# NGoetz/NF

Measured on NVIDIA B200. Metric: nis_flow_fwd_logdet_points_per_sec, higher is better.
Workload: dtype f32

## Files before the change

nf_b200/csrc/flow_fwd.cu:

```cuda
#include <stdlib.h>
#include "common.cuh"
#include "spline.cuh"
#include <cooperative_groups.h>
#include "flow_fwd_common.cuh"

__global__ void flow_pack_kernel(DevFlow F, const float* __restrict__ params, const float* __restrict__ bn_running,
                                 float* __restrict__ wpack, int bn_mode) {
    const int c = blockIdx.y;
    const DevCell& q = F.cells[c];
    const float* p = params + q.param_off;
    float* pk = wpack + q.pk_off;
    const int tid = blockIdx.x * blockDim.x + threadIdx.x, nth = gridDim.x * blockDim.x;
    if (bn_mode == NIS_BN_EVAL) {
        const float* rs = bn_running + q.bn_off;
        for (int l = 0; l <= F.depth; ++l) {
            const int W = F.W(c, l), Wp = F.Wp(c, l);
            const long long g = F.p_bn_gamma(c, l), r = F.r_mean(c, l);
            for (int j = tid; j < Wp; j += nth) {
                float sc = 0.f, sh = 0.f;
                if (j < W) {
                    sc = p[g + j] / sqrtf(rs[r + W + j] + F.eps);
                    sh = p[g + W + j] - rs[r + j] * sc;
                }
                pk[q.aff_off[l] + j] = sc;
// ... 196 lines not shown
template <int NT>
__global__ void __launch_bounds__(NT) flow_fwd_coop_kernel(const __grid_constant__ DevFlow F, const FwdArgs A0) {
    extern __shared__ __align__(16) float sm[];
    cooperative_groups::grid_group grid = cooperative_groups::this_grid();
    const long long rows = A0.B * (F.d + 1);
    FwdArgs A = A0;
    for (int c = 0; c < F.n_cells; ++c) {
        A.c_begin = c; A.c_end = c + 1;
        A.from_state = c > 0;
        A.state_in = c > 0 ? (A0.saved ? A0.saved + (long long)c * rows : A0.scratch_state) : nullptr;
        A.state_out = nullptr; A.to_out = 0;
        for (int l = 0; l <= F.depth; ++l) {
            A.stats_layer = l;
            fwd_generic_body<NT>(F, A, sm);
            grid.sync();
        }
        const bool last = c == F.n_cells - 1;
        A.stats_layer = -1;
        A.to_out = last;
        A.state_out = A0.saved ? A0.saved + (long long)(c + 1) * rows : (last ? nullptr : A0.scratch_state);
        fwd_generic_body<NT>(F, A, sm);
    }
}

size_t nis_flow_bwd_scratch_floats(const DevFlow& F, int64_t B);
bool nis_tiled_supported(const DevFlow& F, int64_t B);
size_t nis_tiled_zbuf_floats(int64_t B);
bool nis_tc_supported(const DevFlow& F, int64_t B, int bn_mode);
int nis_tc_pack(const DevFlow& F, const float* params, float* tcpack, cudaStream_t s);
int nis_launch_tc(const DevFlow& F, const FwdArgs& A, const float* tcpack, cudaStream_t s);
bool nis_tc_split_eval(const DevFlow& F);
bool nis_h_supported(const DevFlow& F, int64_t B, int bn_mode);
int nis_h_pack(const DevFlow& F, const float* params, float* tcpack, cudaStream_t s);
int nis_launch_h(const DevFlow& F, const FwdArgs& A, const float* tcpack, cudaStream_t s);
bool nis_bwd_tc_supported(const DevFlow& F, int64_t B, int bn_mode);
bool nis_wide_supported(const DevFlow& F, int64_t B, int bn_mode);
int nis_wide_pack(const DevFlow& F, const float* params, float* widepack, cudaStream_t s);
int nis_launch_wide(const DevFlow& F, const FwdArgs& A, const float* widepack, cudaStream_t s);
static size_t zbuf_floats(const DevFlow& F, int64_t B) { return nis_tiled_zbuf_floats(B) / 64 * (size_t)(F.maxW > 64 ? F.maxW : 64); }
size_t nis_bwd_tc_scratch_floats(const DevFlow& F, int64_t B);
bool nis_bwd_wide_supported(const DevFlow& F, int64_t B, int bn_mode);
size_t nis_bwd_wide_scratch_floats(const DevFlow& F, int64_t B);
int nis_launch_tiled(const DevFlow& F, const FwdArgs& A, cudaStream_t s);
int nis_launch_col_stats(const DevFlow& F, const FwdArgs& A, cudaStream_t s);
bool nis_moments_supported(const DevFlow& F, int c);
int nis_launch_col_moments(const DevFlow& F, const FwdArgs& A, cudaStream_t s);

#define NIS_TIMING_MAX 512
struct TimingSink { bool on; int n; cudaEvent_t ev[NIS_TIMING_MAX + 1]; int tag[NIS_TIMING_MAX]; bool made; };
static thread_local TimingSink g_timing = {false, 0, {}, {}, false};
static inline void timing_mark(cudaStream_t s, int tag) {
    TimingSink& T = g_timing;
    if (!T.on || T.n >= NIS_TIMING_MAX) return;
    if (tag >= 0) T.tag[T.n++] = tag;
    cudaEventRecord(T.ev[T.n], s);
}
extern "C" int nis_flow_timing_begin(void* stream) {
    TimingSink& T = g_timing;
    if (!T.made) {
        for (int i = 0; i <= NIS_TIMING_MAX; ++i) if (cudaEventCreate(&T.ev[i]) != cudaSuccess) return NIS_ECUDA;
        T.made = true;
    }
    T.on = true; T.n = 0;
    cudaEventRecord(T.ev[0], (cudaStream_t)stream);
    return NIS_OK;
}
extern "C" int nis_flow_timing_end(float* ms, int32_t* tags, int32_t max_n) {
// ... 126 lines not shown
    nis_flow_carve(F, B, workspace, &ws);
    cudaMemsetAsync(ws.counter, 0, 256, s);
    {
        int mx = 0;
        for (int c = 0; c < F.n_cells; ++c) {
            int sz = (c + 1 < F.n_cells ? F.cells[c + 1].pk_off : F.pack_total) - F.cells[c].pk_off;
            if (sz > mx) mx = sz;
        }
        int bx = (mx + 255) / 256;
        if (bx > 64) bx = 64;
        timing_mark(s, -1);
        flow_pack_kernel<<<dim3(bx, F.n_cells), 256, 0, s>>>(F, params, bn_running, ws.wpack, bn_mode);
        NIS_CUDA_CHECK_LAUNCH();
        timing_mark(s, 0);
    }
    FwdArgs A;
    A.in = xj_in; A.in_dtype = in_dtype; A.in_cols = in_cols;
    A.out = xj_out; A.out_dtype = out_dtype;
    A.saved = saved; A.bins = bins_out;
    A.params = params; A.wpack = ws.wpack; A.bn_running = bn_running; A.bn_saved = bn_saved;
    A.partials = ws.partials; A.counter = ws.counter; A.B = B;
    A.zin = nullptr; A.zout = nullptr; A.no_stats = 0; A.z1out = nullptr; A.scratch_state = nullptr; A.inverse = 0; A.zin_layer = 0; A.next_moments = 0;
    const bool tc = nis_tc_supported(F, B, bn_mode);
    const bool hp = tc && nis_h_supported(F, B, bn_mode);
    const bool wide = !tc && nis_wide_supported(F, B, bn_mode);
    const bool tiled = tc || wide || nis_tiled_supported(F, B);
    static const int recompute_env = [] { const char* e = getenv("NIS_TRAIN_RECOMPUTE"); return e ? (e[0] == '1' ? 1 : 0) : -1; }();
    const bool recompute = hp && (recompute_env >= 0 ? recompute_env == 1 : false);
    static const int skip_env = [] { const char* e = getenv("NIS_SKIP_LAST_STORE"); return e && e[0] == '0' ? 0 : 1; }();
    const bool skip_last = hp && !recompute && skip_env && F.depth >= 3 && F.kind == NIS_KIND_PWLIN;
    if (tc) { rc = hp ? nis_h_pack(F, params, ws.tcpack, s) : nis_tc_pack(F, params, ws.tcpack, s); if (rc) return rc; timing_mark(s, 0); }
    if (wide) { rc = nis_wide_pack(F, params, ws.tcpack, s); if (rc) return rc; }
    const long long rows = (long long)B * (F.d + 1);
    if (bn_mode == NIS_BN_EVAL && !tiled) {
        A.state_in = nullptr; A.state_out = nullptr; A.from_state = 0; A.to_out = 1;
        A.c_begin = 0; A.c_end = F.n_cells; A.stats_layer = -1;
        return launch_fwd_any(F, A, s);
    }
    if (bn_mode == NIS_BN_TRAIN && !tiled) {
        static const int coop_env = [] { const char* e = getenv("NIS_COOP"); return e && e[0] == '0' ? 0 : 1; }();
        if (coop_env) {
            A.scratch_state = ws.state;
            A.state_in = nullptr; A.state_out = nullptr; A.from_state = 0; A.to_out = 0;
            A.c_begin = 0; A.c_end = 1; A.stats_layer = 0;
            rc = launch_fwd_coop(F, A, s);
            if (rc == NIS_OK) { timing_mark(s, 2); return NIS_OK; }
        }
    }
    static const int fuse_env = [] { const char* e = getenv("NIS_FUSE_MOMENTS"); return e && e[0] == '0' ? 0 : 1; }();
    bool moments_ready = false;
    float* acts = (wide && bn_mode == NIS_BN_TRAIN && act_saved && saved && nis_act_cache_floats(F, B)) ? act_saved : nullptr;
    const size_t act_layer = (size_t)((B + 127) / 128) * (size_t)F.widths[0] * 128;
    for (int c = 0; c < F.n_cells; ++c) {
        A.c_begin = c; A.c_end = c + 1;
        A.from_state = c > 0;
        A.state_in = c > 0 ? (saved ? saved + (long long)c * rows : ws.state) : nullptr;
        A.state_out = nullptr; A.to_out = 0;
        float* zb[2] = {ws.bwd, ws.bwd + zbuf_floats(F, B)};
        float* const acell = acts ? acts + (size_t)c * F.depth * act_layer : nullptr;
        const bool moments = tiled && bn_mode == NIS_BN_TRAIN && nis_moments_supported(F, c);
        if (bn_mode == NIS_BN_TRAIN) {
            int l0 = 0;
            if (moments) {
                if (!moments_ready) {
                    A.stats_layer = 0;
                    rc = nis_launch_col_moments(F, A, s);
                    if (rc) return rc;
                    timing_mark(s, 1);
                }
                l0 = 2;
            }
            for (int l = l0; l <= F.depth; ++l) {
                A.stats_layer = l;
                if (tiled && l >= 1) {
                    A.zin = (l >= 2 && !(moments && l == 2) && !recompute) ? zb[(l - 1) & 1] : nullptr;
                    A.zout = (recompute || (skip_last && moments && l == F.depth)) ? nullptr : zb[l & 1];
                    if (acell) {
                        if (A.zin) A.zin = acell + (size_t)(l - 2) * act_layer;
                        A.zout = acell + (size_t)(l - 1) * act_layer;
                        A.z1out = (!A.zin && l == 2) ? acell : nullptr;
                    }
                    rc = hp ? nis_launch_h(F, A, ws.tcpack, s) : tc ? nis_launch_tc(F, A, ws.tcpack, s)
                            : wide ? nis_launch_wide(F, A, ws.tcpack, s) : nis_launch_tiled(F, A, s);
                } else if (tiled && l == 0) {
                    rc = nis_launch_col_stats(F, A, s);
                } else {
                    rc = launch_fwd_any(F, A, s);
                }
                if (rc) return rc;
                timing_mark(s, (tc || wide) && l >= 1 ? 10 + 1 + (A.zin ? 2 : 0) : 2);
            }
        }
        A.stats_layer = -1;
        A.zin = (tiled && bn_mode == NIS_BN_TRAIN && !(moments && F.depth == 1) && !recompute) ? zb[F.depth & 1] : nullptr;
        A.zout = nullptr;
        if (acell) { A.zin = acell + (size_t)(F.depth - 1) * act_layer; A.z1out = nullptr; }
        if (skip_last && moments && bn_mode == NIS_BN_TRAIN) { A.zin = zb[(F.depth - 1) & 1]; A.zin_layer = F.depth - 1; }
        if (tc && !hp && bn_mode == NIS_BN_EVAL && nis_tc_split_eval(F)) {
            A.stats_layer = F.depth; A.no_stats = 1; A.zin = nullptr; A.zout = zb[F.depth & 1];
            rc = nis_launch_tc(F, A, ws.tcpack, s);
            if (rc) return rc;
            A.stats_layer = -1; A.no_stats = 0; A.zin = zb[F.depth & 1]; A.zout = nullptr;
        }
        if (wide && bn_mode == NIS_BN_EVAL) {
            A.no_stats = 1;
            for (int l = 2; l <= F.depth; ++l) {
                A.stats_layer = l;
                A.zin = l > 2 ? zb[(l - 1) & 1] : nullptr;
                A.zout = zb[l & 1];
                rc = nis_launch_wide(F, A, ws.tcpack, s);
                if (rc) return rc;
            }
            A.stats_layer = -1; A.no_stats = 0; A.zin = F.depth >= 2 ? zb[F.depth & 1] : nullptr; A.zout = nullptr;
        }
        const bool last = c == F.n_cells - 1;
        A.next_moments = hp && fuse_env && bn_mode == NIS_BN_TRAIN && !last && A.zin != nullptr
                         && nis_moments_supported(F, c + 1) && F.cells[c + 1].P <= 4;
        moments_ready = A.next_moments != 0;
        A.to_out = last;
        A.state_out = saved ? saved + (long long)(c + 1) * rows : (last ? nullptr : ws.state);
        rc = hp ? nis_launch_h(F, A, ws.tcpack, s) : tc ? nis_launch_tc(F, A, ws.tcpack, s) : wide ? nis_launch_wide(F, A, ws.tcpack, s)
                : (tiled ? nis_launch_tiled(F, A, s) : launch_fwd_any(F, A, s));
        if (rc) return rc;
        timing_mark(s, (tc || wide) ? 10 + (A.zin ? 2 : 0) : 2);
        A.zin_layer = 0;
    }
    return NIS_OK;
}

extern "C" int nis_flow_inverse(const NisFlowDesc* desc, const float* params, const float* bn_running,
                                const void* yj_in, int32_t in_dtype, int32_t in_cols,
                                void* xj_out, int32_t out_dtype, int32_t* bins_out, int32_t bn_mode,
                                void* workspace, size_t workspace_bytes, int64_t B, void* stream) {
    DevFlow F;
    int rc = nis_build_dev_flow(desc, &F);
    if (rc) return rc;
    if (!params || !workspace || B < 0 || (B > 0 && (!yj_in || !xj_out))) return NIS_EINVAL;
    if (in_cols != F.d && in_cols != F.d + 1) return NIS_EINVAL;
    if ((in_dtype != NIS_F32 && in_dtype != NIS_F64) || (out_dtype != NIS_F32 && out_dtype != NIS_F64)) return NIS_EINVAL;
    if (bn_mode == NIS_BN_EVAL && !bn_running) return NIS_EINVAL;
    if (workspace_bytes < nis_flow_workspace_bytes(desc, B)) return NIS_EWORKSPACE;
    if (B == 0) return NIS_OK;
    cudaStream_t s = (cudaStream_t)stream;
    FlowWorkspace ws;
    nis_flow_carve(F, B, workspace, &ws);
    cudaMemsetAsync(ws.counter, 0, 256, s);
    {
        int mx = 0;
        for (int c = 0; c < F.n_cells; ++c) {
            int sz = (c + 1 < F.n_cells ? F.cells[c + 1].pk_off : F.pack_total) - F.cells[c].pk_off;
            if (sz > mx) mx = sz;
        }
        int bx = (mx + 255) / 256;
        if (bx > 64) bx = 64;
        flow_pack_kernel<<<dim3(bx, F.n_cells), 256, 0, s>>>(F, params, bn_running, ws.wpack, bn_mode);
        NIS_CUDA_CHECK_LAUNCH();
// ... 32 lines not shown
```

nf_b200/csrc/flow_tc_h.cu:

```cuda
#include <stdlib.h>
#include <cuda_fp16.h>
#include "common.cuh"
#include "spline.cuh"
#include "flow_fwd_common.cuh"
#include "tc_common.cuh"
#include "tc_spline.cuh"

#define H_SA 8.0f
#define H_AMAX 65504.0f
#define H_HID_BYTES (2 * TCH * TCH * 2)
#define H_MAXG 4
template <int KIND> struct HK {
    static constexpr int OUT_N = KIND == NIS_KIND_PWLIN ? 64 : 80;
    static constexpr int TPER = KIND == NIS_KIND_PWLIN ? 2 : 1;
    static constexpr int SLOT = KIND == NIS_KIND_PWLIN ? 32 : 80;
    static constexpr int COLS = KIND == NIS_KIND_PWLIN ? 128 : 160;
    static constexpr int COL_AHI = KIND == NIS_KIND_PWLIN ? 64 : 96;
    static constexpr int COL_ALO = COL_AHI + 32;
    static constexpr int MAXG = KIND == NIS_KIND_PWLIN ? 4 : 3;
};
__host__ __device__ static inline int h_slot(const DevFlow& F) { return F.kind == NIS_KIND_PWLIN ? 32 : 80; }
__host__ __device__ static inline int h_out_rows(const DevFlow& F) {
    int mt = 1;
    for (int c = 0; c < F.n_cells; ++c) mt = F.cells[c].T > mt ? F.cells[c].T : mt;
// ... 42 lines not shown
    const int rows_src = outl ? q.T * F.K : TCH, rows = outl ? h_out_rows(F) : TCH, slot = h_slot(F);
    float m = 0.f;
    for (int i = tid; i < rows_src * kin; i += 256) m = fmaxf(m, fabsf(w[i]));
#pragma unroll
    for (int o = 16; o > 0; o >>= 1) m = fmaxf(m, __shfl_xor_sync(0xffffffffu, m, o));
    if ((tid & 31) == 0) red[tid >> 5] = m;
    __syncthreads();
    if (tid == 0) {
        for (int i = 1; i < 8; ++i) m = fmaxf(m, red[i]);
        int e = 14;
        if (m > 0.f && m < 3.0e38f) frexpf(m, &e);
        e = e < -100 ? -100 : (e > 100 ? 100 : e);
        sw_s = ldexpf(1.f, 14 - e);
    }
    __syncthreads();
    const float SW = sw_s;
    char* dst = hpack + (size_t)c * h_cell_bytes(F);
    char* hi = dst + (first ? h_l0_off(F) : (size_t)li * H_HID_BYTES);
    char* lo = hi + (size_t)rows * TCH * 2;
    for (int i = tid; i < rows * TCH; i += 256) {
        const int n = i / TCH, k = i - n * TCH;
        const int t = outl ? n / slot : 0, jj = outl ? n - t * slot : n;
        const bool live = outl ? (t < q.T && jj < F.K) : k < kin;
        const float v = live ? w[(size_t)(outl ? t * F.K + jj : n) * kin + k] * SW : 0.f;
        const __half h = __float2half_rn(v);
        const int o = h_off(n, k);
        *reinterpret_cast<__half*>(hi + o) = h;
        *reinterpret_cast<__half*>(lo + o) = __float2half_rn(v - __half2float(h));
    }
    if (tid == 0) reinterpret_cast<float*>(dst + h_cell_bytes(F) - 64)[l] = 1.f / (H_SA * SW);
}

struct HSmem {
    int w0, aff, bias, st, sst, red, zb, total;
    int wfirst;
    __host__ __device__ int wl(int l) const { return (l - wfirst) * H_HID_BYTES; }
};
__host__ __device__ static inline HSmem h_layout(const DevFlow& F, int P, int l_begin, int l_end, bool zstage, int NG,
                                                 bool layer0 = true, bool stats = true) {
    HSmem s;
    int o = 0;
    s.wfirst = l_begin > 1 ? l_begin : 1;
    for (int l = s.wfirst; l <= l_end; ++l) o += l == F.depth ? h_out_bytes(F) : H_HID_BYTES;
    (void)P;
    s.w0 = o; o += layer0 ? H_HID_BYTES : 0;
    s.aff = o; o += (F.depth + 1) * 2 * TCH * 4;
    s.bias = o; o += h_out_rows(F) * 4;
    s.st = o; o += NG * (F.d + 1) * TCM * 4;
    o = (o + 15) & ~15;
    s.sst = o; o += NG * (F.d + 1) * TCM * 4;
    o = (o + 7) & ~7;
    s.red = o; o += stats ? (NG * TCM * 2 + 2 * F.maxW) * 8 : 0;
    o = (o + 127) & ~127;
    s.zb = o;
    if (zstage) o += NG * TCH * TCM * 4;
    s.total = o;
    return s;
}

__device__ __forceinline__ void h_store_act32(const float* v, const float* sc, const float* sh, uint32_t t_hi, uint32_t t_lo) {
    uint32_t hi[16], lo[16];
#pragma unroll
    for (int j4 = 0; j4 < 8; ++j4) {
        const float4 s4 = reinterpret_cast<const float4*>(sc)[j4], h4 = reinterpret_cast<const float4*>(sh)[j4];
        const float a0 = fmaxf(fmaf(v[4 * j4], s4.x, h4.x), 0.f), a1 = fmaxf(fmaf(v[4 * j4 + 1], s4.y, h4.y), 0.f);
        const float a2 = fmaxf(fmaf(v[4 * j4 + 2], s4.z, h4.z), 0.f), a3 = fmaxf(fmaf(v[4 * j4 + 3], s4.w, h4.w), 0.f);
        const uint32_t p01 = h_pack_sat(a0, a1), p23 = h_pack_sat(a2, a3);
        const float2 f01 = __half22float2(*reinterpret_cast<const __half2*>(&p01));
        const float2 f23 = __half22float2(*reinterpret_cast<const __half2*>(&p23));
        hi[2 * j4] = p01;
        hi[2 * j4 + 1] = p23;
        lo[2 * j4] = h_pack_sat(a0 - f01.x, a1 - f01.y);
        lo[2 * j4 + 1] = h_pack_sat(a2 - f23.x, a3 - f23.y);
    }
    tc_st16(t_hi, hi);
    tc_st16(t_lo, lo);
}

__device__ __forceinline__ void h_issue_block(uint32_t tmem_d, uint32_t t_hi, uint32_t t_lo, uint32_t w_hi, uint32_t w_lo, uint32_t idesc) {
#pragma unroll
    for (int ks = 0; ks < 4; ++ks) {
        h_mma_ts(tmem_d, t_hi + ks * 8, tc_desc(w_lo + ks * 32), idesc, ks > 0);
        h_mma_ts(tmem_d, t_lo + ks * 8, tc_desc(w_hi + ks * 32), idesc, 1);
    }
#pragma unroll
    for (int ks = 0; ks < 4; ++ks) h_mma_ts(tmem_d, t_hi + ks * 8, tc_desc(w_hi + ks * 32), idesc, 1);
}

template <int NG, int KIND, int MODE>
__global__ void __launch_bounds__(NG * TCM, 1) flow_cell_h_kernel(const __grid_constant__ DevFlow F, const FwdArgs A,
                                                                        const char* __restrict__ hpack) {
    constexpr int NT = NG * TCM;
    typedef HK<KIND> K_;
    constexpr int H_COLS = K_::COLS, H_COL_AHI = K_::COL_AHI, H_COL_ALO = K_::COL_ALO;
    extern __shared__ char smraw[];
    __shared__ uint64_t a_ready[NG], d_ready[NG], z_full[NG], s_full[NG];
    __shared__ uint32_t tmem_base_s;
    char* sm = smem_align1024(smraw);
    const int tid = threadIdx.x, warp = tid >> 5, lane = tid & 31;
    const int c = A.c_begin;
    const DevCell& q = F.cells[c];
    const int d = F.d, depth = F.depth;
    constexpr bool stats = (MODE & 1) != 0;
    constexpr bool from_z = (MODE & 2) != 0;
    constexpr bool nextmom = (MODE & 4) != 0;
    constexpr bool needs_state = !(from_z && stats);
    constexpr int MOM_N = 4 + 4 * 5 / 2;
    float macc[nextmom ? MOM_N : 1];
#pragma unroll
    for (int i = 0; i < (nextmom ? MOM_N : 1); ++i) macc[i] = 0.f;
    const int lz = from_z ? (A.zin_layer > 0 ? A.zin_layer : (stats ? A.stats_layer - 1 : depth)) : 1;
    const int l_end = stats ? A.stats_layer - 1 : depth;
    const bool zst = from_z || stats;
    const HSmem L = h_layout(F, q.P, lz, l_end, zst, NG, !from_z, stats);
    float* affs = reinterpret_cast<float*>(sm + L.aff);
    float* biass = reinterpret_cast<float*>(sm + L.bias);
    const float* pk = A.wpack + q.pk_off;
    const char* cellpack = hpack + (size_t)c * h_cell_bytes(F);
    const float* inv_scale = reinterpret_cast<const float*>(cellpack + h_cell_bytes(F) - 64);

    for (int l = L.wfirst; l <= l_end; ++l) {
        const int n16 = (l == depth ? h_out_bytes(F) : H_HID_BYTES) / 16;
        const uint4* src = reinterpret_cast<const uint4*>(cellpack + (size_t)(l - 1) * H_HID_BYTES);
        uint4* dst = reinterpret_cast<uint4*>(sm + L.wl(l));
        for (int i = tid; i < n16; i += NT) dst[i] = src[i];
    }
    if (!from_z) {
        const uint4* src = reinterpret_cast<const uint4*>(cellpack + h_l0_off(F));
        uint4* dst = reinterpret_cast<uint4*>(sm + L.w0);
        for (int i = tid; i < H_HID_BYTES / 16; i += NT) dst[i] = src[i];
    }
    for (int l = 0; l <= depth; ++l) {
        const int W = l == 0 ? q.P : TCH, Wp = pad8(W);
        const float* s = pk + q.aff_off[l];
        const float f = H_SA;
        const float fs = (l >= 1 && l >= lz && l <= l_end) ? f * inv_scale[l - 1] : f;
        for (int i = tid; i < W; i += NT) { affs[l * 2 * TCH + i] = fs * s[i]; affs[l * 2 * TCH + TCH + i] = f * s[Wp + i]; }
    }
    const int out_rows = h_out_rows(F);
    constexpr float LOGIT_UNIT = 1.4426950408889634f;
    for (int i = tid; i < out_rows; i += NT) {
        const int t = i / K_::SLOT, jj = i - t * K_::SLOT;
        biass[i] = (t < q.T && jj < F.K) ? LOGIT_UNIT * pk[q.bo_off + t * F.Kpad + jj] : 0.f;
    }
    if (tid == 0) {
        for (int g = 0; g < NG; ++g) {
            mbar_init(&a_ready[g], TCM); mbar_init(&d_ready[g], 1); mbar_init(&z_full[g], 1); mbar_init(&s_full[g], 1);
        }
        asm volatile("fence.mbarrier_init.release.cluster;" ::: "memory");
    }
    if (warp == 0) {
        asm volatile("tcgen05.alloc.cta_group::1.sync.aligned.shared::cta.b32 [%0], %1;" ::"r"(smem_u32(&tmem_base_s)), "r"(512));
        asm volatile("tcgen05.relinquish_alloc_permit.cta_group::1.sync.aligned;" ::);
    }
    proxy_fence();
    tc_fence_before();
    __syncthreads();
    tc_fence_after();
    const uint32_t tmem_base = tmem_base_s;
    const long long ntiles = (A.B + TCM - 1) / TCM;
    const long long rowlen = d + 1;
    const int nblk = (q.T + K_::TPER - 1) / K_::TPER;
    const bool has_out = l_end == depth;
    double dsum = 0.0, dsq = 0.0;

    const uint32_t idesc = h_idesc(TCM, TCH), idesc_out = h_idesc(TCM, K_::OUT_N);
    {
        const int g = warp >> 2, gt = tid & (TCM - 1);
        float* st = reinterpret_cast<float*>(sm + L.st) + g * (d + 1) * TCM + gt;
        const uint32_t tg = tmem_base + g * H_COLS + ((uint32_t)((warp & 3) * 32) << 16);
        uint32_t pd = 0, pa = 0, zph = 0, sph = 0;
        float* zs = reinterpret_cast<float*>(sm + L.zb) + g * TCH * TCM;
        constexpr uint32_t ZBYTES = TCH * TCM * 4;
        float* sst = reinterpret_cast<float*>(sm + L.sst) + g * (d + 1) * TCM;
        const uint32_t SBYTES = (uint32_t)((d + 1) * TCM * 4);
        const bool st_bulk = needs_state && A.from_state && (reinterpret_cast<uintptr_t>(A.state_in) & 15) == 0 && (SBYTES & 15) == 0;
        if (st_bulk && gt == 0) {
            const long long t0 = (long long)blockIdx.x * NG + g;
            if ((t0 + 1) * TCM <= A.B) bulk_load(sst, A.state_in + t0 * TCM * rowlen, SBYTES, &s_full[g]);
        }
        const float inv_out = has_out ? LOGIT_UNIT * inv_scale[depth] : 0.f;
        for (long long it = 0;; ++it) {
            const long long tile = ((long long)blockIdx.x + it * gridDim.x) * NG + g;
            if (tile >= ntiles) break;
            const long long tn = tile + (long long)gridDim.x * NG;
            if (from_z && gt == 0) {
                if (A.zout) bulk_store_wait_read();
                bulk_load(zs, A.zin + (size_t)tile * TCH * TCM, ZBYTES, &z_full[g]);
                if (tn < ntiles) bulk_prefetch_l2(A.zin + (size_t)tn * TCH * TCM, ZBYTES);
            }
            const long long pt = tile * TCM + gt;
            const bool valid = pt < A.B;
            if (!needs_state) {
            } else if (st_bulk && (tile + 1) * TCM <= A.B) {
                mbar_wait(&s_full[g], sph);
                sph ^= 1;
                for (int i = 0; i <= d; ++i) st[i * TCM] = sst[gt * rowlen + i];
                proxy_fence();
                group_sync(g);
                if (gt == 0 && (tn + 1) * TCM <= A.B) bulk_load(sst, A.state_in + tn * TCM * rowlen, SBYTES, &s_full[g]);
            } else if (valid) {
                if (A.from_state) {
                    for (int i = 0; i <= d; ++i) st[i * TCM] = A.state_in[pt * rowlen + i];
                } else {
                    for (int i = 0; i < d; ++i) st[i * TCM] = load_io(A.in, A.in_dtype, pt * A.in_cols + i);
                    st[d * TCM] = A.in_cols > d ? load_io(A.in, A.in_dtype, pt * A.in_cols + d) : 1.f;
                }
                if (!stats && A.saved && !A.from_state) {
                    float* sv = A.saved + ((long long)c * A.B + pt) * rowlen;
                    for (int i = 0; i <= d; ++i) sv[i] = st[i * TCM];
                }
            } else {
                for (int i = 0; i < d; ++i) st[i * TCM] = 0.5f;
                st[d * TCM] = 1.f;
            }
            if (from_z) { mbar_wait(&z_full[g], zph); zph ^= 1; }
            if (!from_z) {
                uint32_t hi[8], lo[8];
#pragma unroll
// ... 23 lines not shown
                }
                pa ^= 1;
                mbar_wait(&d_ready[g], pd);
                pd ^= 1;
                tc_fence_after();
            }
            for (int l = lz; l <= l_end; ++l) {
                const float* sc = affs + l * 2 * TCH;
#pragma unroll 1
                for (int h = 0; h < 2; ++h) {
                    float v[32];
                    if (l > lz || !from_z) {
                        tc_ld32(tg + 32 * h, v);
                        tc_ld_wait();
                    } else {
                        const float* zr = zs + (32 * h) * TCM + gt;
#pragma unroll
                        for (int j = 0; j < 32; ++j) v[j] = zr[j * TCM];
                    }
                    h_store_act32(v, sc + 32 * h, sc + TCH + 32 * h, tg + H_COL_AHI + 16 * h, tg + H_COL_ALO + 16 * h);
                }
                if (l == lz && from_z) proxy_fence();
                tc_st_wait();
                tc_fence_before();
                mbar_arrive(&a_ready[g]);
                if (gt == 0) {
                    mbar_wait(&a_ready[g], pa);
                    tc_fence_after();
                    const uint32_t whi = smem_u32(sm + L.wl(l));
                    const uint32_t tb = tmem_base + g * H_COLS;
                    h_issue_block(tb, tb + H_COL_AHI, tb + H_COL_ALO, whi, whi + (l == depth ? out_rows : TCH) * TCH * 2,
                                  l == depth ? idesc_out : idesc);
                    tc_commit(&d_ready[g]);
                }
                pa ^= 1;
                if (l < depth) {
                    mbar_wait(&d_ready[g], pd);
                    pd ^= 1;
                    tc_fence_after();
                }
            }
            if (stats) {
                if (!from_z) {
                    if (gt == 0) bulk_store_wait_read();
                    group_sync(g);
                }
                const bool full = (tile + 1) * TCM <= A.B;
#pragma unroll 1
                for (int h = 0; h < 2; ++h) {
                    float v[32];
                    tc_ld32(tg + 32 * h, v);
                    tc_ld_wait();
                    if (full) {
#pragma unroll
                        for (int j = 0; j < 32; ++j) zs[(32 * h + j) * TCM + gt] = v[j];
                    } else {
#pragma unroll
                        for (int j = 0; j < 32; ++j) zs[(32 * h + j) * TCM + gt] = valid ? v[j] : 0.f;
                    }
                }
                proxy_fence();
                group_sync(g);
                if (gt == 0 && A.zout) bulk_store(A.zout + (size_t)tile * TCH * TCM, zs, ZBYTES);
                if (!A.no_stats) {
                    const float4* row = reinterpret_cast<const float4*>(zs + (gt & 63) * TCM + (gt >> 6) * 64);
                    float s_ = 0.f, q_ = 0.f;
#pragma unroll
                    for (int i = 0; i < 16; ++i) {
                        const float4 x = row[(i + lane) & 15];
                        s_ += (x.x + x.y) + (x.z + x.w);
                        q_ = fmaf(x.x, x.x, fmaf(x.y, x.y, fmaf(x.z, x.z, fmaf(x.w, x.w, q_))));
                    }
                    dsum += (double)s_; dsq += (double)q_;
// ... 126 lines not shown
    if (warp == 0) asm volatile("tcgen05.dealloc.cta_group::1.sync.aligned.b32 %0, %1;" ::"r"(tmem_base), "r"(512));
    if (nextmom) {
        __shared__ bool s_last_m;
        __shared__ double sc0s_m[4 + 16];
        double* redm = reinterpret_cast<double*>(sm + L.zb);
        double* totm = redm + (NT / 32) * MOM_N;
#pragma unroll
        for (int i = 0; i < MOM_N; ++i) {
            double a = (double)macc[i];
#pragma unroll
            for (int o = 16; o > 0; o >>= 1) a += __shfl_xor_sync(0xffffffffu, a, o);
            if (lane == 0) redm[warp * MOM_N + i] = a;
        }
        __syncthreads();
        if (tid < MOM_N) {
            double s_ = 0.0;
            for (int w = 0; w < NT / 32; ++w) s_ += redm[w * MOM_N + tid];
            A.partials[(size_t)blockIdx.x * MOM_N + tid] = s_;
        }
        __threadfence();
        __syncthreads();
        if (tid == 0) s_last_m = atomicAdd(A.counter, 1u) == gridDim.x - 1;
        __syncthreads();
        if (!s_last_m) return;
        __threadfence();
        fold_partials<MOM_N>(A.partials, gridDim.x, totm + MOM_N, totm, tid, NT);
        moments_finalize<4>(F, A, c + 1, totm, sc0s_m, tid, NT);
        if (tid == 0) *A.counter = 0u;
        return;
    }
    if (!stats || A.no_stats) return;
    double* red = reinterpret_cast<double*>(sm + L.red);
    double* sacc = red + NG * TCM * 2;
    red[tid] = dsum; red[NG * TCM + tid] = dsq;
    for (int i = tid; i < 2 * F.maxW; i += NT) sacc[i] = 0.0;
    __syncthreads();
    if (tid < TCH) {
        double s = 0.0, s2 = 0.0;
        for (int k = 0; k < 2 * NG; ++k) { s += red[tid + 64 * k]; s2 += red[NG * TCM + tid + 64 * k]; }
        const double k1 = (double)inv_scale[l_end];
        sacc[tid] = s * k1; sacc[F.maxW + tid] = s2 * k1 * k1;
    }
    bn_stats_finalize(F, A, sacc, NT, red);
}

size_t nis_h_pack_floats(const DevFlow& F) {
    if (F.depth < 1) return 0;
    return (size_t)F.n_cells * (h_cell_bytes(F) / 4);
}

int64_t nis_tc_min_batch(int64_t dflt);

static int h_groups(const DevFlow& F) {
    const size_t lim = 226 * 1024;
    for (int ng = F.kind == NIS_KIND_PWLIN ? HK<NIS_KIND_PWLIN>::MAXG : HK<NIS_KIND_PWQUAD>::MAXG; ng >= 2; --ng) {
        bool ok = true;
        for (int c = 0; c < F.n_cells && ok; ++c) {
            const int P = F.cells[c].P;
            ok = (size_t)h_layout(F, P, 1, F.depth, false, ng).total + 1024 <= lim
                 && (size_t)h_layout(F, P, F.depth - 1, F.depth - 1, true, ng).total + 1024 <= lim
                 && (size_t)h_layout(F, P, F.depth, F.depth, true, ng, false, false).total + 1024 <= lim
                 && (F.depth < 3 || (size_t)h_layout(F, P, F.depth - 1, F.depth, true, ng, false, false).total + 1024 <= lim);
        }
        if (ok) return ng;
    }
    return 0;
}

bool nis_h_supported(const DevFlow& F, int64_t B, int bn_mode) {
    (void)bn_mode;
    const char* off = getenv("NIS_TC_H");
    if (off && off[0] == '0') return false;
    const char* tcoff = getenv("NIS_TC");
    if (tcoff && tcoff[0] == '0') return false;
    if (F.nb != 32 || F.depth < 1 || F.maxW != TCH) return false;
    if (F.kind == NIS_KIND_PWLIN ? F.K != 32 : F.K != 65) return false;
    if (B < nis_tc_min_batch(256)) return false;
    for (int l = 0; l < F.depth; ++l) if (F.widths[l] != TCH) return false;
    for (int c = 0; c < F.n_cells; ++c)
        if (F.cells[c].P > 16 || (F.kind == NIS_KIND_PWLIN && F.cells[c].T * 32 > 128)) return false;
    return h_groups(F) >= 2;
}

int nis_h_pack(const DevFlow& F, const float* params, float* tcpack, cudaStream_t s) {
    flow_h_pack_kernel<<<dim3(F.depth + 1, F.n_cells), 256, 0, s>>>(F, params, reinterpret_cast<char*>(tcpack));
    NIS_CUDA_CHECK_LAUNCH();
    return NIS_OK;
}

template <int NG, int KIND, int MODE>
static int h_launch_mode(const DevFlow& F, const FwdArgs& A, const char* hpack, size_t smem, int sms, cudaStream_t s) {
    static int attr_smem = 0;
    if ((int)smem > attr_smem) {
        if (cudaFuncSetAttribute(flow_cell_h_kernel<NG, KIND, MODE>, cudaFuncAttributeMaxDynamicSharedMemorySize, (int)smem) != cudaSuccess)
            return NIS_ECUDA;
        attr_smem = (int)smem;
    }
    const long long nsets = ((A.B + TCM - 1) / TCM + NG - 1) / NG;
    const int grid = (int)(nsets < sms ? nsets : sms);
    flow_cell_h_kernel<NG, KIND, MODE><<<grid, NG * TCM, smem, s>>>(F, A, hpack);
    NIS_CUDA_CHECK_LAUNCH();
    return NIS_OK;
}

template <int NG, int KIND>
static int h_launch(const DevFlow& F, const FwdArgs& A, const char* hpack, size_t smem, int sms, cudaStream_t s) {
    switch ((A.stats_layer >= 1 ? 1 : 0) | (A.zin != nullptr ? 2 : 0)) {
        case 0: return h_launch_mode<NG, KIND, 0>(F, A, hpack, smem, sms, s);
        case 1: return h_launch_mode<NG, KIND, 1>(F, A, hpack, smem, sms, s);
        case 2: return A.next_moments ? h_launch_mode<NG, KIND, 6>(F, A, hpack, smem, sms, s)
                                      : h_launch_mode<NG, KIND, 2>(F, A, hpack, smem, sms, s);
    }
    return h_launch_mode<NG, KIND, 3>(F, A, hpack, smem, sms, s);
}

int nis_launch_h(const DevFlow& F, const FwdArgs& A, const float* tcpack, cudaStream_t s) {
    static int sms = 0;
    if (sms <= 0) {
        int dev = 0;
        cudaGetDevice(&dev);
        cudaDeviceGetAttribute(&sms, cudaDevAttrMultiProcessorCount, dev);
        if (sms <= 0) sms = 148;
    }
    const bool stats = A.stats_layer >= 1;
    const int lz = A.zin ? (A.zin_layer > 0 ? A.zin_layer : (stats ? A.stats_layer - 1 : F.depth)) : 1;
    const int l_end = stats ? A.stats_layer - 1 : F.depth;
    const int ng = h_groups(F);
    const size_t smem = (size_t)h_layout(F, F.cells[A.c_begin].P, lz, l_end, A.zin != nullptr || stats, ng, A.zin == nullptr, stats).total + 1024;
    const char* hp = reinterpret_cast<const char*>(tcpack);
    if (F.kind == NIS_KIND_PWLIN) {
        switch (ng) {
            case 4: return h_launch<4, NIS_KIND_PWLIN>(F, A, hp, smem, sms, s);
            case 3: return h_launch<3, NIS_KIND_PWLIN>(F, A, hp, smem, sms, s);
            case 2: return h_launch<2, NIS_KIND_PWLIN>(F, A, hp, smem, sms, s);
        }
    } else {
        switch (ng) {
            case 3: return h_launch<3, NIS_KIND_PWQUAD>(F, A, hp, smem, sms, s);
            case 2: return h_launch<2, NIS_KIND_PWQUAD>(F, A, hp, smem, sms, s);
        }
    }
    return NIS_EUNSUPPORTED;
}
```

nf_b200/csrc/tc_common.cuh:

```cuda
#pragma once
#include <cuda_runtime.h>
#include <stdint.h>
#include "common.cuh"

#define TCM 128
#define TCH 64
#define TC_KT 32
#define TC_NOUT 128

__device__ __forceinline__ float tf32_rn(float a) {
    return __uint_as_float((__float_as_uint(a) + 0x1000u) & 0xFFFFE000u);
}
__device__ __forceinline__ uint32_t smem_u32(const void* p) { return (uint32_t)__cvta_generic_to_shared(p); }

__device__ __forceinline__ char* smem_align1024(char* smraw) { return smraw + ((1024u - (smem_u32(smraw) & 1023u)) & 1023u); }

__device__ __forceinline__ void mbar_init(uint64_t* bar, int count) {
    asm volatile("mbarrier.init.shared::cta.b64 [%0], %1;" ::"r"(smem_u32(bar)), "r"(count));
}
__device__ __forceinline__ void mbar_wait(uint64_t* bar, uint32_t parity) {
    const uint32_t a = smem_u32(bar);
    for (int it = 0; it < (1 << 22); ++it) {
        uint32_t ok;
        asm volatile("{\n\t.reg .pred p;\n\tmbarrier.try_wait.parity.shared::cta.b64 p, [%1], %2;\n\tselp.b32 %0, 1, 0, p;\n\t}"
// ... 14 lines not shown
__device__ __forceinline__ void tc_commit(uint64_t* bar) {
    asm volatile("tcgen05.commit.cta_group::1.mbarrier::arrive::one.shared::cluster.b64 [%0];" ::"r"(smem_u32(bar)) : "memory");
}
__device__ __forceinline__ void tc_fence_before() { asm volatile("tcgen05.fence::before_thread_sync;" ::: "memory"); }
__device__ __forceinline__ void tc_fence_after() { asm volatile("tcgen05.fence::after_thread_sync;" ::: "memory"); }
__device__ __forceinline__ void proxy_fence() { asm volatile("fence.proxy.async.shared::cta;" ::: "memory"); }

__device__ __forceinline__ void tc_mma_tf32_ts(uint32_t tmem_d, uint32_t tmem_a, uint64_t desc_b, uint32_t idesc, uint32_t accumulate) {
    asm volatile(
        "{\n\t.reg .pred p;\n\tsetp.ne.b32 p, %4, 0;\n\t"
        "tcgen05.mma.cta_group::1.kind::tf32 [%0], [%1], %2, %3, p;\n\t}"
        ::"r"(tmem_d), "r"(tmem_a), "l"(desc_b), "r"(idesc), "r"(accumulate) : "memory");
}
__device__ __forceinline__ void tc_mma_tf32_ss(uint32_t tmem_d, uint64_t desc_a, uint64_t desc_b, uint32_t idesc, uint32_t accumulate) {
    asm volatile(
        "{\n\t.reg .pred p;\n\tsetp.ne.b32 p, %4, 0;\n\t"
        "tcgen05.mma.cta_group::1.kind::tf32 [%0], %1, %2, %3, p;\n\t}"
        ::"r"(tmem_d), "l"(desc_a), "l"(desc_b), "r"(idesc), "r"(accumulate) : "memory");
}
__device__ __forceinline__ void bulk_load(void* smem_dst, const void* gmem_src, uint32_t bytes, uint64_t* bar) {
    asm volatile("mbarrier.arrive.expect_tx.shared::cta.b64 _, [%0], %1;" ::"r"(smem_u32(bar)), "r"(bytes) : "memory");
    asm volatile("cp.async.bulk.shared::cluster.global.mbarrier::complete_tx::bytes [%0], [%1], %2, [%3];"
                 ::"r"(smem_u32(smem_dst)), "l"(gmem_src), "r"(bytes), "r"(smem_u32(bar)) : "memory");
}
__device__ __forceinline__ void bulk_store(void* gmem_dst, const void* smem_src, uint32_t bytes) {
    asm volatile("cp.async.bulk.global.shared::cta.bulk_group [%0], [%1], %2;" ::"l"(gmem_dst), "r"(smem_u32(smem_src)), "r"(bytes) : "memory");
    asm volatile("cp.async.bulk.commit_group;" ::: "memory");
}
__device__ __forceinline__ void bulk_store_wait_read() { asm volatile("cp.async.bulk.wait_group.read 0;" ::: "memory"); }
__device__ __forceinline__ void group_sync(int g) { asm volatile("bar.sync %0, %1;" ::"r"(1 + g), "r"(TCM) : "memory"); }
__device__ __forceinline__ void mbar_arrive(uint64_t* bar) {
    asm volatile("mbarrier.arrive.shared::cta.b64 _, [%0];" ::"r"(smem_u32(bar)) : "memory");
}

__device__ __forceinline__ uint64_t tc_desc(uint32_t smem_addr) {
    uint64_t d = 0;
    d |= (uint64_t)((smem_addr >> 4) & 0x3FFF);
    d |= (uint64_t)1 << 16;
    d |= (uint64_t)(1024 >> 4) << 32;
    d |= (uint64_t)1 << 46;
    d |= (uint64_t)2 << 61;
    return d;
}
__host__ __device__ constexpr uint32_t tc_idesc(int M, int N) {
    return (1u << 4) | (2u << 7) | (2u << 10) | ((uint32_t)(N >> 3) << 17) | ((uint32_t)(M >> 4) << 24);
}

__host__ __device__ static inline int tc_off(int rows, int row, int k) {
    const int kt = k >> 5, kk = k & 31;
    return kt * rows * 128 + (row >> 3) * 1024 + (row & 7) * 128 + ((((kk >> 2) ^ (row & 7)) << 4) | ((kk & 3) << 2));
}

__host__ __device__ static inline int tc_slab_off(int rows, int row, int p) {
    return (p >> 5) * rows * 128 + (row >> 3) * 1024 + (row & 7) * 128 + (((((p & 31) >> 2) ^ (row & 7)) << 4) | ((p & 3) << 2));
}

__host__ __device__ static inline int tc_out_n(const DevFlow& F) { return F.K == 32 ? 128 : 80; }
__host__ __device__ static inline int tc_out_tper(const DevFlow& F) { return F.K == 32 ? 4 : 1; }
__host__ __device__ static inline int tc_out_slot(const DevFlow& F) { return F.K == 32 ? 32 : 80; }
__host__ __device__ static inline int tc_out_blocks(const DevFlow& F, int T) { return (T + tc_out_tper(F) - 1) / tc_out_tper(F); }
__host__ __device__ static inline int tc_max_blocks(const DevFlow& F) {
    int m = 1;
    for (int c = 0; c < F.n_cells; ++c) { const int b = tc_out_blocks(F, F.cells[c].T); m = b > m ? b : m; }
    return m;
}
__host__ __device__ static inline int tc_cell_floats(const DevFlow& F) {
// ... 149 lines not shown
```

Measured before the change: 618.2 million.

## Add PDL launch overlap and early z-prefetch stats path to H kernel

```diff
diff --git a/nf_b200/csrc/flow_fwd.cu b/nf_b200/csrc/flow_fwd.cu
--- a/nf_b200/csrc/flow_fwd.cu
+++ b/nf_b200/csrc/flow_fwd.cu
@@ -252,7 +252,7 @@
 bool nis_tc_split_eval(const DevFlow& F);
 bool nis_h_supported(const DevFlow& F, int64_t B, int bn_mode);
 int nis_h_pack(const DevFlow& F, const float* params, float* tcpack, cudaStream_t s);
-int nis_launch_h(const DevFlow& F, const FwdArgs& A, const float* tcpack, cudaStream_t s);
+int nis_launch_h(const DevFlow& F, const FwdArgs& A, const float* tcpack, bool pdl, cudaStream_t s);
 bool nis_bwd_tc_supported(const DevFlow& F, int64_t B, int bn_mode);
 bool nis_wide_supported(const DevFlow& F, int64_t B, int bn_mode);
 int nis_wide_pack(const DevFlow& F, const float* params, float* widepack, cudaStream_t s);
@@ -445,6 +445,7 @@
     if (tc) { rc = hp ? nis_h_pack(F, params, ws.tcpack, s) : nis_tc_pack(F, params, ws.tcpack, s); if (rc) return rc; timing_mark(s, 0); }
     if (wide) { rc = nis_wide_pack(F, params, ws.tcpack, s); if (rc) return rc; }
     const long long rows = (long long)B * (F.d + 1);
+    bool pdl = false;
     if (bn_mode == NIS_BN_EVAL && !tiled) {
         A.state_in = nullptr; A.state_out = nullptr; A.from_state = 0; A.to_out = 1;
         A.c_begin = 0; A.c_end = F.n_cells; A.stats_layer = -1;
@@ -480,6 +481,7 @@
                     rc = nis_launch_col_moments(F, A, s);
                     if (rc) return rc;
                     timing_mark(s, 1);
+                    pdl = hp;
                 }
                 l0 = 2;
             }
@@ -493,7 +495,7 @@
                         A.zout = acell + (size_t)(l - 1) * act_layer;
                         A.z1out = (!A.zin && l == 2) ? acell : nullptr;
                     }
-                    rc = hp ? nis_launch_h(F, A, ws.tcpack, s) : tc ? nis_launch_tc(F, A, ws.tcpack, s)
+                    rc = hp ? nis_launch_h(F, A, ws.tcpack, pdl, s) : tc ? nis_launch_tc(F, A, ws.tcpack, s)
                             : wide ? nis_launch_wide(F, A, ws.tcpack, s) : nis_launch_tiled(F, A, s);
                 } else if (tiled && l == 0) {
                     rc = nis_launch_col_stats(F, A, s);
@@ -501,6 +503,7 @@
                     rc = launch_fwd_any(F, A, s);
                 }
                 if (rc) return rc;
+                pdl = hp;
                 timing_mark(s, (tc || wide) && l >= 1 ? 10 + 1 + (A.zin ? 2 : 0) : 2);
             }
         }
@@ -532,9 +535,10 @@
         moments_ready = A.next_moments != 0;
         A.to_out = last;
         A.state_out = saved ? saved + (long long)(c + 1) * rows : (last ? nullptr : ws.state);
-        rc = hp ? nis_launch_h(F, A, ws.tcpack, s) : tc ? nis_launch_tc(F, A, ws.tcpack, s) : wide ? nis_launch_wide(F, A, ws.tcpack, s)
+        rc = hp ? nis_launch_h(F, A, ws.tcpack, pdl, s) : tc ? nis_launch_tc(F, A, ws.tcpack, s) : wide ? nis_launch_wide(F, A, ws.tcpack, s)
                 : (tiled ? nis_launch_tiled(F, A, s) : launch_fwd_any(F, A, s));
         if (rc) return rc;
+        pdl = hp;
         timing_mark(s, (tc || wide) ? 10 + (A.zin ? 2 : 0) : 2);
         A.zin_layer = 0;
     }
diff --git a/nf_b200/csrc/flow_tc_h.cu b/nf_b200/csrc/flow_tc_h.cu
--- a/nf_b200/csrc/flow_tc_h.cu
+++ b/nf_b200/csrc/flow_tc_h.cu
@@ -98,12 +98,12 @@
 }
 
 struct HSmem {
-    int w0, aff, bias, st, sst, red, zb, total;
+    int w0, aff, bias, st, sst, red, zb, zh, total;
     int wfirst;
     __host__ __device__ int wl(int l) const { return (l - wfirst) * H_HID_BYTES; }
 };
 __host__ __device__ static inline HSmem h_layout(const DevFlow& F, int P, int l_begin, int l_end, bool zstage, int NG,
-                                                 bool layer0 = true, bool stats = true) {
+                                                 bool layer0 = true, bool stats = true, bool state = true, bool zhalf = false) {
     HSmem s;
     int o = 0;
     s.wfirst = l_begin > 1 ? l_begin : 1;
@@ -112,14 +112,16 @@
     s.w0 = o; o += layer0 ? H_HID_BYTES : 0;
     s.aff = o; o += (F.depth + 1) * 2 * TCH * 4;
     s.bias = o; o += h_out_rows(F) * 4;
-    s.st = o; o += NG * (F.d + 1) * TCM * 4;
+    s.st = o; o += state ? NG * (F.d + 1) * TCM * 4 : 0;
     o = (o + 15) & ~15;
-    s.sst = o; o += NG * (F.d + 1) * TCM * 4;
+    s.sst = o; o += state ? NG * (F.d + 1) * TCM * 4 : 0;
     o = (o + 7) & ~7;
     s.red = o; o += stats ? (NG * TCM * 2 + 2 * F.maxW) * 8 : 0;
     o = (o + 127) & ~127;
     s.zb = o;
     if (zstage) o += NG * TCH * TCM * 4;
+    s.zh = o;
+    if (zhalf) o += NG * (TCH / 2) * TCM * 4;
     s.total = o;
     return s;
 }
@@ -178,7 +180,8 @@
     const int lz = from_z ? (A.zin_layer > 0 ? A.zin_layer : (stats ? A.stats_layer - 1 : depth)) : 1;
     const int l_end = stats ? A.stats_layer - 1 : depth;
     const bool zst = from_z || stats;
-    const HSmem L = h_layout(F, q.P, lz, l_end, zst, NG, !from_z, stats);
+    const bool early_z = from_z && (!stats || A.zout == nullptr);
+    const HSmem L = h_layout(F, q.P, lz, l_end, zst, NG, !from_z, stats, needs_state, stats && early_z);
     float* affs = reinterpret_cast<float*>(sm + L.aff);
     float* biass = reinterpret_cast<float*>(sm + L.bias);
     const float* pk = A.wpack + q.pk_off;
@@ -196,6 +199,18 @@
         uint4* dst = reinterpret_cast<uint4*>(sm + L.w0);
         for (int i = tid; i < H_HID_BYTES / 16; i += NT) dst[i] = src[i];
     }
+    if (tid == 0) {
+        for (int g = 0; g < NG; ++g) {
+            mbar_init(&a_ready[g], TCM); mbar_init(&d_ready[g], 1); mbar_init(&z_full[g], 1); mbar_init(&s_full[g], 1);
+        }
+        asm volatile("fence.mbarrier_init.release.cluster;" ::: "memory");
+    }
+    if (warp == 0) {
+        asm volatile("tcgen05.alloc.cta_group::1.sync.aligned.shared::cta.b32 [%0], %1;" ::"r"(smem_u32(&tmem_base_s)), "r"(512));
+        asm volatile("tcgen05.relinquish_alloc_permit.cta_group::1.sync.aligned;" ::);
+    }
+    grid_dep_wait();
+    grid_dep_launch();
     for (int l = 0; l <= depth; ++l) {
         const int W = l == 0 ? q.P : TCH, Wp = pad8(W);
         const float* s = pk + q.aff_off[l];
@@ -208,16 +223,6 @@
     for (int i = tid; i < out_rows; i += NT) {
         const int t = i / K_::SLOT, jj = i - t * K_::SLOT;
         biass[i] = (t < q.T && jj < F.K) ? LOGIT_UNIT * pk[q.bo_off + t * F.Kpad + jj] : 0.f;
-    }
-    if (tid == 0) {
-        for (int g = 0; g < NG; ++g) {
-            mbar_init(&a_ready[g], TCM); mbar_init(&d_ready[g], 1); mbar_init(&z_full[g], 1); mbar_init(&s_full[g], 1);
-        }
-        asm volatile("fence.mbarrier_init.release.cluster;" ::: "memory");
-    }
-    if (warp == 0) {
-        asm volatile("tcgen05.alloc.cta_group::1.sync.aligned.shared::cta.b32 [%0], %1;" ::"r"(smem_u32(&tmem_base_s)), "r"(512));
-        asm volatile("tcgen05.relinquish_alloc_permit.cta_group::1.sync.aligned;" ::);
     }
     proxy_fence();
     tc_fence_before();
@@ -245,12 +250,20 @@
             const long long t0 = (long long)blockIdx.x * NG + g;
             if ((t0 + 1) * TCM <= A.B) bulk_load(sst, A.state_in + t0 * TCM * rowlen, SBYTES, &s_full[g]);
         }
+        if (early_z && gt == 0) {
+            const long long t0 = (long long)blockIdx.x * NG + g;
+            if (t0 < ntiles) {
+                bulk_load(zs, A.zin + (size_t)t0 * TCH * TCM, ZBYTES, &z_full[g]);
+                const long long t1 = t0 + (long long)gridDim.x * NG;
+                if (t1 < ntiles) bulk_prefetch_l2(A.zin + (size_t)t1 * TCH * TCM, ZBYTES);
+            }
+        }
         const float inv_out = has_out ? LOGIT_UNIT * inv_scale[depth] : 0.f;
         for (long long it = 0;; ++it) {
             const long long tile = ((long long)blockIdx.x + it * gridDim.x) * NG + g;
             if (tile >= ntiles) break;
             const long long tn = tile + (long long)gridDim.x * NG;
-            if (from_z && gt == 0) {
+            if (from_z && !early_z && gt == 0) {
                 if (A.zout) bulk_store_wait_read();
                 bulk_load(zs, A.zin + (size_t)tile * TCH * TCM, ZBYTES, &z_full[g]);
                 if (tn < ntiles) bulk_prefetch_l2(A.zin + (size_t)tn * TCH * TCM, ZBYTES);
@@ -340,6 +353,11 @@
                     h_issue_block(tb, tb + H_COL_AHI, tb + H_COL_ALO, whi, whi + (l == depth ? out_rows : TCH) * TCH * 2,
                                   l == depth ? idesc_out : idesc);
                     tc_commit(&d_ready[g]);
+                    if (early_z && l == lz && tn < ntiles) {
+                        bulk_load(zs, A.zin + (size_t)tn * TCH * TCM, ZBYTES, &z_full[g]);
+                        const long long tp = tn + (long long)gridDim.x * NG;
+                        if (tp < ntiles) bulk_prefetch_l2(A.zin + (size_t)tp * TCH * TCM, ZBYTES);
+                    }
                 }
                 pa ^= 1;
                 if (l < depth) {
@@ -347,6 +365,38 @@
                     pd ^= 1;
                     tc_fence_after();
                 }
+            }
+            if (stats && early_z) {
+                float* zh = reinterpret_cast<float*>(sm + L.zh) + g * (TCH / 2) * TCM;
+                const bool full = (tile + 1) * TCM <= A.B;
+#pragma unroll 1
+                for (int h = 0; h < 2; ++h) {
+                    float v[32];
+                    tc_ld32(tg + 32 * h, v);
+                    tc_ld_wait();
+                    if (h) group_sync(g);
+                    if (full) {
+#pragma unroll
+                        for (int j = 0; j < 32; ++j) zh[j * TCM + gt] = v[j];
+                    } else {
+#pragma unroll
+                        for (int j = 0; j < 32; ++j) zh[j * TCM + gt] = valid ? v[j] : 0.f;
+                    }
+                    group_sync(g);
+                    if (!A.no_stats && (gt >> 6) == h) {
+                        const float4* row = reinterpret_cast<const float4*>(zh + (gt & 31) * TCM + ((gt >> 5) & 1) * 64);
+                        float s_ = 0.f, q_ = 0.f;
+#pragma unroll
+                        for (int i = 0; i < 16; ++i) {
+                            const float4 x = row[(i + lane) & 15];
+                            s_ += (x.x + x.y) + (x.z + x.w);
+                            q_ = fmaf(x.x, x.x, fmaf(x.y, x.y, fmaf(x.z, x.z, fmaf(x.w, x.w, q_))));
+                        }
+                        dsum += (double)s_; dsq += (double)q_;
+                    }
+                }
+                group_sync(g);
+                continue;
             }
             if (stats) {
                 if (!from_z) {
@@ -539,7 +589,8 @@
     if (!stats || A.no_stats) return;
     double* red = reinterpret_cast<double*>(sm + L.red);
     double* sacc = red + NG * TCM * 2;
-    red[tid] = dsum; red[NG * TCM + tid] = dsq;
+    const int slot = (from_z && early_z) ? (tid & ~96) | ((tid & 32) << 1) | ((tid & 64) >> 1) : tid;
+    red[slot] = dsum; red[NG * TCM + slot] = dsq;
     for (int i = tid; i < 2 * F.maxW; i += NT) sacc[i] = 0.0;
     __syncthreads();
     if (tid < TCH) {
@@ -566,6 +617,7 @@
             const int P = F.cells[c].P;
             ok = (size_t)h_layout(F, P, 1, F.depth, false, ng).total + 1024 <= lim
                  && (size_t)h_layout(F, P, F.depth - 1, F.depth - 1, true, ng).total + 1024 <= lim
+                 && (size_t)h_layout(F, P, F.depth - 1, F.depth - 1, true, ng, false, true, false, true).total + 1024 <= lim
                  && (size_t)h_layout(F, P, F.depth, F.depth, true, ng, false, false).total + 1024 <= lim
                  && (F.depth < 3 || (size_t)h_layout(F, P, F.depth - 1, F.depth, true, ng, false, false).total + 1024 <= lim);
         }
@@ -596,7 +648,7 @@
 }
 
 template <int NG, int KIND, int MODE>
-static int h_launch_mode(const DevFlow& F, const FwdArgs& A, const char* hpack, size_t smem, int sms, cudaStream_t s) {
+static int h_launch_mode(const DevFlow& F, const FwdArgs& A, const char* hpack, size_t smem, int sms, bool pdl, cudaStream_t s) {
     static int attr_smem = 0;
     if ((int)smem > attr_smem) {
         if (cudaFuncSetAttribute(flow_cell_h_kernel<NG, KIND, MODE>, cudaFuncAttributeMaxDynamicSharedMemorySize, (int)smem) != cudaSuccess)
@@ -605,23 +657,33 @@
     }
     const long long nsets = ((A.B + TCM - 1) / TCM + NG - 1) / NG;
     const int grid = (int)(nsets < sms ? nsets : sms);
-    flow_cell_h_kernel<NG, KIND, MODE><<<grid, NG * TCM, smem, s>>>(F, A, hpack);
+    cudaLaunchAttribute attr;
+    attr.id = cudaLaunchAttributeProgrammaticStreamSerialization;
+    attr.val.programmaticStreamSerializationAllowed = 1;
+    cudaLaunchConfig_t cfg = {};
+    cfg.gridDim = dim3(grid);
+    cfg.blockDim = dim3(NG * TCM);
+    cfg.dynamicSmemBytes = smem;
+    cfg.stream = s;
+    cfg.attrs = &attr;
+    cfg.numAttrs = pdl ? 1 : 0;
+    if (cudaLaunchKernelEx(&cfg, flow_cell_h_kernel<NG, KIND, MODE>, F, A, hpack) != cudaSuccess) return NIS_ECUDA;
     NIS_CUDA_CHECK_LAUNCH();
     return NIS_OK;
 }
 
 template <int NG, int KIND>
-static int h_launch(const DevFlow& F, const FwdArgs& A, const char* hpack, size_t smem, int sms, cudaStream_t s) {
+static int h_launch(const DevFlow& F, const FwdArgs& A, const char* hpack, size_t smem, int sms, bool pdl, cudaStream_t s) {
     switch ((A.stats_layer >= 1 ? 1 : 0) | (A.zin != nullptr ? 2 : 0)) {
-        case 0: return h_launch_mode<NG, KIND, 0>(F, A, hpack, smem, sms, s);
-        case 1: return h_launch_mode<NG, KIND, 1>(F, A, hpack, smem, sms, s);
-        case 2: return A.next_moments ? h_launch_mode<NG, KIND, 6>(F, A, hpack, smem, sms, s)
-                                      : h_launch_mode<NG, KIND, 2>(F, A, hpack, smem, sms, s);
-    }
-    return h_launch_mode<NG, KIND, 3>(F, A, hpack, smem, sms, s);
-}
-
-int nis_launch_h(const DevFlow& F, const FwdArgs& A, const float* tcpack, cudaStream_t s) {
+        case 0: return h_launch_mode<NG, KIND, 0>(F, A, hpack, smem, sms, pdl, s);
+        case 1: return h_launch_mode<NG, KIND, 1>(F, A, hpack, smem, sms, pdl, s);
+        case 2: return A.next_moments ? h_launch_mode<NG, KIND, 6>(F, A, hpack, smem, sms, pdl, s)
+                                      : h_launch_mode<NG, KIND, 2>(F, A, hpack, smem, sms, pdl, s);
+    }
+    return h_launch_mode<NG, KIND, 3>(F, A, hpack, smem, sms, pdl, s);
+}
+
+int nis_launch_h(const DevFlow& F, const FwdArgs& A, const float* tcpack, bool pdl, cudaStream_t s) {
     static int sms = 0;
     if (sms <= 0) {
         int dev = 0;
@@ -633,18 +695,20 @@
     const int lz = A.zin ? (A.zin_layer > 0 ? A.zin_layer : (stats ? A.stats_layer - 1 : F.depth)) : 1;
     const int l_end = stats ? A.stats_layer - 1 : F.depth;
     const int ng = h_groups(F);
-    const size_t smem = (size_t)h_layout(F, F.cells[A.c_begin].P, lz, l_end, A.zin != nullptr || stats, ng, A.zin == nullptr, stats).total + 1024;
+    const bool from_z = A.zin != nullptr, stats_only = from_z && stats && A.zout == nullptr;
+    const size_t smem = (size_t)h_layout(F, F.cells[A.c_begin].P, lz, l_end, from_z || stats, ng, !from_z, stats,
+                                         !(from_z && stats), stats_only).total + 1024;
     const char* hp = reinterpret_cast<const char*>(tcpack);
     if (F.kind == NIS_KIND_PWLIN) {
         switch (ng) {
-            case 4: return h_launch<4, NIS_KIND_PWLIN>(F, A, hp, smem, sms, s);
-            case 3: return h_launch<3, NIS_KIND_PWLIN>(F, A, hp, smem, sms, s);
-            case 2: return h_launch<2, NIS_KIND_PWLIN>(F, A, hp, smem, sms, s);
+            case 4: return h_launch<4, NIS_KIND_PWLIN>(F, A, hp, smem, sms, pdl, s);
+            case 3: return h_launch<3, NIS_KIND_PWLIN>(F, A, hp, smem, sms, pdl, s);
+            case 2: return h_launch<2, NIS_KIND_PWLIN>(F, A, hp, smem, sms, pdl, s);
         }
     } else {
         switch (ng) {
-            case 3: return h_launch<3, NIS_KIND_PWQUAD>(F, A, hp, smem, sms, s);
-            case 2: return h_launch<2, NIS_KIND_PWQUAD>(F, A, hp, smem, sms, s);
+            case 3: return h_launch<3, NIS_KIND_PWQUAD>(F, A, hp, smem, sms, pdl, s);
+            case 2: return h_launch<2, NIS_KIND_PWQUAD>(F, A, hp, smem, sms, pdl, s);
         }
     }
     return NIS_EUNSUPPORTED;
diff --git a/nf_b200/csrc/tc_common.cuh b/nf_b200/csrc/tc_common.cuh
--- a/nf_b200/csrc/tc_common.cuh
+++ b/nf_b200/csrc/tc_common.cuh
@@ -70,6 +70,8 @@
 __device__ __forceinline__ void mbar_arrive(uint64_t* bar) {
     asm volatile("mbarrier.arrive.shared::cta.b64 _, [%0];" ::"r"(smem_u32(bar)) : "memory");
 }
+__device__ __forceinline__ void grid_dep_wait() { asm volatile("griddepcontrol.wait;" ::: "memory"); }
+__device__ __forceinline__ void grid_dep_launch() { asm volatile("griddepcontrol.launch_dependents;" ::: "memory"); }
 
 __device__ __forceinline__ uint64_t tc_desc(uint32_t smem_addr) {
     uint64_t d = 0;
```

After: 609.8 million, median of 6. -1.4%, worse.
